# zraorg/ZRA

Measured on AMD Instinct MI355X. Metric: compress + RA-decompress GiB/s, 16 GiB @ 64 KiB frames, 1/2/4/8 MI355X, higher is better.
Workload: dtype u8

## Files before the change

zra_amd/csrc/zra_decode.hip:

```cpp
#include "zra_dev.h"
#include "zra_kernels.h"

using namespace zra_dev;

namespace {

constexpr int DEC_THREADS = 64;
constexpr int BATCH = 64;
#ifndef ZRA_XWIN
#define ZRA_XWIN 4032
#endif
constexpr u32 XPRE = 64, XWIN = ZRA_XWIN;
constexpr u32 BLOCK_MAX = 128u << 10;

__constant__ u32 c_ll_base[36] = {0,1,2,3,4,5,6,7,8,9,10,11,12,13,14,15,16,18,20,22,24,28,32,40,48,64,128,256,512,1024,2048,4096,8192,16384,32768,65536};
__constant__ u8 c_ll_bits[36] = {0,0,0,0,0,0,0,0,0,0,0,0,0,0,0,0,1,1,1,1,2,2,3,3,4,6,7,8,9,10,11,12,13,14,15,16};
__constant__ u32 c_ml_base[53] = {3,4,5,6,7,8,9,10,11,12,13,14,15,16,17,18,19,20,21,22,23,24,25,26,27,28,29,30,31,32,33,34,
                                  35,37,39,41,43,47,51,59,67,83,99,131,259,515,1027,2051,4099,8195,16387,32771,65539};
__constant__ u8 c_ml_bits[53] = {0,0,0,0,0,0,0,0,0,0,0,0,0,0,0,0,0,0,0,0,0,0,0,0,0,0,0,0,0,0,0,0,
                                 1,1,1,1,2,2,3,3,4,4,5,7,8,9,10,11,12,13,14,15,16};
__constant__ short c_ll_defnorm[36] = {4,3,2,2,2,2,2,2,2,2,2,2,2,1,1,1,2,2,2,2,2,2,2,2,2,3,2,1,1,1,1,1,-1,-1,-1,-1};
__constant__ short c_ml_defnorm[53] = {1,4,3,2,2,2,2,2,2,1,1,1,1,1,1,1,1,1,1,1,1,1,1,1,1,1,1,1,1,1,1,1,
                                       1,1,1,1,1,1,1,1,1,1,1,1,1,1,-1,-1,-1,-1,-1,-1,-1};
__constant__ short c_of_defnorm[29] = {1,1,1,1,1,1,2,2,2,1,1,1,1,1,1,1,1,1,1,1,1,1,1,1,-1,-1,-1,-1,-1};
__constant__ u16 c_huf_t0[16][2] = {{0,0},{0,0},{38,130},{448,128},{556,128},{714,128},{883,128},{897,128},{926,128},{947,128},{1107,128},{1177,128},{1242,128},{1349,128},{1455,128},{722,128}};
__constant__ u16 c_huf_t1[16][2] = {{1,1},{1,1},{1313,74},{1353,74},{1353,74},{1418,74},{1437,74},{1515,75},{1613,75},{1729,77},{2083,81},{2379,87},{2415,93},{2644,106},{2422,124},{1891,145}};

__device__ __forceinline__ u64 mk_seqsym(u32 baseValue, u32 addBits, u32 nbBits, u32 nextBase) {
  return (u64)baseValue | ((u64)addBits << 32) | ((u64)nbBits << 40) | ((u64)nextBase << 48);
}
__device__ __forceinline__ u32 mk_cell(u32 sym, u32 addBits, u32 nbBits, u32 nextBase) {
  return sym | (addBits << 8) | (nbBits << 16) | (nextBase << 20);
}

#ifdef ZRA_SMALL_PROFILE
__device__ unsigned long long zra_small_prof[64];
extern "C" __attribute__((visibility("default"))) void ZraHipDebugReadSmallProfile(unsigned long long* out16, int reset) {
  (void)hipMemcpyFromSymbol(out16, HIP_SYMBOL(zra_small_prof), sizeof(unsigned long long) * 64);
  if (reset) { unsigned long long z[64] = {0}; (void)hipMemcpyToSymbol(HIP_SYMBOL(zra_small_prof), z, sizeof(z)); }
}
#define SPROF(k) { __builtin_amdgcn_s_waitcnt(0); const u64 n_ = __builtin_amdgcn_s_memtime(); if (lane == 0) atomicAdd(&zra_small_prof[k], n_ - spt_); spt_ = n_; }
#define SPROF_T0 u64 spt_ = __builtin_amdgcn_s_memtime();
#define SPROF_RESET spt_ = __builtin_amdgcn_s_memtime();
#else
#define SPROF(k)
#define SPROF_T0
#define SPROF_RESET
#endif
#ifdef ZRA_SMALL_PROFILE
#define PPROF_T0 u64 ppt_ = __builtin_amdgcn_s_memtime();
#define PPROF(k) if (FUSED) { __builtin_amdgcn_s_waitcnt(0); const u64 n_ = __builtin_amdgcn_s_memtime(); if (lane == 0) atomicAdd(&zra_small_prof[k], n_ - ppt_); ppt_ = n_; }
#define LPROF_T0 u64 lpt_ = __builtin_amdgcn_s_memtime();
#define LPROF(k) { __builtin_amdgcn_s_waitcnt(0); const u64 n_ = __builtin_amdgcn_s_memtime(); atomicAdd(&zra_small_prof[k], n_ - lpt_); lpt_ = n_; }
#else
#define PPROF_T0
#define PPROF(k)
#define LPROF_T0
#define LPROF(k)
#endif
constexpr u32 STAGE_BYTES = 512;
struct __attribute__((aligned(16))) ParseShared {
  u8 w0[STAGE_BYTES + 16];
  u8 w1[STAGE_BYTES + 16];
  union {
    u64 wt[64];
    u32 stage[1024];
  };
  u16 wnext[256];
  short norm[256];
  u8 spread[512];
  u8 weights[256];
  u16 hufStart[256];
  u32 rankStart[16];
  u32 err, job;
  u32 blkType, blkSize, blkLast, blkPos, hdrPos, frameEnd, winPos, winLen;
  u32 litType, litRegen, litComp, litHdr, litStreams, litRle;
  u32 hufValid, hufMaxBits, hufNSym, hufX2;
  u32 hufNw, hufUsed, hufPhase;
  u32 hufTl, hufMaxSym, hufNcBytes, hufHbyte;
  u32 nbSeq, seqPos, seqModes, seqTables;
  u32 llLog, mlLog, ofLog, llValid, mlValid, ofValid, ofShare;
  u32 rep[3];
  u32 streamOff[4], streamLen[4];
// ... 1185 lines not shown
    const u32 v = (u32)((c << (bc & 63)) >> ((64 - nb) & 63));
    bc += nb; return v;
  }
  __device__ __forceinline__ int reload() {
    if (bc > 64) return OVERFLOW;
    if (ptr >= 8) { ptr -= bc >> 3; bc &= 7; c = fetch(ptr); return UNFINISHED; }
    if (ptr == 0) return bc < 64 ? ENDOFBUFFER : COMPLETED;
    u32 nbBytes = bc >> 3; int r = UNFINISHED;
    if (ptr < nbBytes) { nbBytes = ptr; r = ENDOFBUFFER; }
    ptr -= nbBytes; bc -= nbBytes * 8; c = fetch(ptr);
    return r;
  }
  __device__ __forceinline__ void reload_quiet(bool wide, const u8* pad) {
    const u32 nb = bc <= 64 ? min(bc >> 3, ptr) : 0u;
    ptr -= nb; bc -= nb * 8;
    const u64 v = RING ? fetch(ptr) : ld64(wide ? base + ptr : pad);
    c = nb ? v : c;
  }
};
typedef ZdsT<false> Zds;

}

namespace {
template <bool LDSTAB>
__device__ __forceinline__ void chain_body(const ZraDecodeArgs& a, u32* const ldsTabs, u32* const baseLL, u32* const baseML, u32* const ldsRings = nullptr) {
  const int lane = threadIdx.x;
  const u32 nPend = a.counters[ZRA_DC_NPENDING];
  bool have = false, drained = false;
  ZraDecFrame* F = nullptr;
  const u32* T = nullptr;
  u64* sq = nullptr;
  ZdsT<LDSTAB> br; br.c = 0; br.bc = 0; br.ptr = 0; br.base = nullptr; br.ring = nullptr; br.rLo = 0;
  br.lim = a.body + a.bodySize; br.pf = make_uint4(0, 0, 0, 0); br.pfState = 0; br.pfAge = 0;
  if (LDSTAB) br.ring = (u8*)(ldsRings + (u32)lane * CHAIN_RING_WORDS);
  u32 sLL = 0, sOF = 0, sML = 0, rep0 = 1, rep1 = 4, rep2 = 8;
  u32 i = 0, nbSeq = 0, outPos = 0, litPos = 0, outCap = 0, regen = 0, produced0 = 0, limit = 0;
  u32 longMode = 0, err = 0, jErr = 0xFFFFFFFFu, valid = 0, validOut = 0, validLit = 0, truncated = 0;
  u64 q0 = 0, q1 = 0, q2 = 0;
  u32 eL = 0, eM = 0, eO = 0;
  bool wide = false; const u8* pad = nullptr;
  bool fresh = false; u32 freshJob = 0;
  const u16* const cells16 = (const u16*)ldsTabs + (size_t)lane * ZRA_DEC_TBL_WORDS;
  u32 logLL = 0, logML = 0, logOF = 0;
  auto fetch_cells = [&]() {
    if (LDSTAB) { eL = cells16[ZRA_DEC_TBL_LL + sLL]; eM = cells16[ZRA_DEC_TBL_ML + sML]; eO = cells16[ZRA_DEC_TBL_OF + sOF]; }
    else { eL = T[ZRA_DEC_TBL_LL + sLL]; eM = T[ZRA_DEC_TBL_ML + sML]; eO = T[ZRA_DEC_TBL_OF + sOF]; }
  };
  auto c_code = [&](u32 e) -> u32 { return e & 63u; };
  auto c_sbits = [&](u32 e, u32 lg) -> u32 { if (LDSTAB) return lg - (31u - (u32)__builtin_clz(e >> 6)); return (e >> 16) & 0xF; };
  auto c_sbase = [&](u32 e, u32 lg) -> u32 {
    if (LDSTAB) { const u32 v = e >> 6, hb = 31u - (u32)__builtin_clz(v); return (v ^ (1u << hb)) << (lg - hb); }
    return e >> 20;
  };
  baseLL[lane] = lane < 36 ? c_ll_base[lane] | (LDSTAB ? (u32)c_ll_bits[lane] << 24 : 0u) : 0u;
  baseML[lane] = lane < 53 ? c_ml_base[lane] | (LDSTAB ? (u32)c_ml_bits[lane] << 24 : 0u) : 0u;
  wsync();
  if (LDSTAB && (u32)lane >= ZRA_CHAIN_LDS_FRAMES) drained = true;

  auto finish = [&]() {
    { const u32 r = valid & 3u, b = valid - r;
      if (r >= 1) sq[b] = q0;
      if (r >= 2) sq[b + 1] = q1;
      if (r >= 3) sq[b + 2] = q2; }
    if (!err && !truncated) {
      if (regen - litPos > outCap - outPos) err = ZE_DSTSIZE_TOOSMALL;
    }
    F->chainErr = err; F->nSeqValid = valid; F->seqOut = validOut; F->seqLit = validLit; F->truncated = truncated;
    F->repOut[0] = rep0; F->repOut[1] = rep1; F->repOut[2] = rep2;
    have = false;
  };

  for (;;) {
    const u64 want = __ballot(!have && !drained);
    if (want) {
      u32 base = 0;
      const u32 cnt = (u32)__builtin_popcountll(want);
      if (lane == (int)__builtin_ctzll(want)) base = atomicAdd(&a.counters[ZRA_DC_QCHAIN], cnt);
      base = bcast_u32(base, (u32)__builtin_ctzll(want));
      if (!have && !drained) {
        const u32 idx = base + (u32)__builtin_popcountll(want & ((1ull << lane) - 1ull));
        if (idx >= nPend) drained = true;
        else {
          const u32 j = a.pending[idx];
          const size_t gj = frame_of(a, j);
          F = &a.frames[j];
          T = a.tables + (size_t)j * ZRA_DEC_TBL_WORDS;
          const u8* const blk = a.body + a.frameOff[gj * a.offStride] + F->bpos;
          nbSeq = F->nbSeq; regen = F->litRegen; produced0 = F->produced; longMode = F->longMode;
          outCap = a.outCap[gj] - produced0;
          limit = a.limit ? a.limit[gj] : 0xFFFFFFFFu;
          sq = a.seqs + F->seqBase;
          rep0 = F->rep[0]; rep1 = F->rep[1]; rep2 = F->rep[2];
          i = 0; outPos = 0; litPos = 0; err = 0; jErr = 0xFFFFFFFFu; valid = 0; validOut = 0; validLit = 0; truncated = 0;
          have = true; br.rLo = 0; br.pfState = 0;
          if (F->hufErr) { err = ZE_CORRUPTION; nbSeq = 0; finish(); }
          else if (F->lateErr) { err = F->lateErr; nbSeq = 0; finish(); }
          else if (nbSeq) {
            if (!br.init(blk + F->seqPos, F->bsize - F->seqPos)) { err = ZE_CORRUPTION; finish(); }
            else {
              logLL = F->llLog; logOF = F->ofLog; logML = F->mlLog;
              sLL = br.read(logLL); br.reload();
              sOF = br.read(logOF); br.reload();
              sML = br.read(logML); br.reload();
              wide = F->bsize - F->seqPos >= 8;
              pad = a.body + a.frameOff[gj * a.offStride];
              if (LDSTAB) { fresh = true; freshJob = j; } else fetch_cells();
            }
          }
        }
      }
    }
    if (LDSTAB) {
      u64 nm = __ballot(fresh);
      while (nm) {
        const u32 l = (u32)__builtin_ctzll(nm); nm &= nm - 1;
        const u32 jj = bcast_u32(freshJob, l);
        const uint4* const g4 = (const uint4*)(a.tables + (size_t)jj * ZRA_DEC_TBL_WORDS);
        uint2* const d2 = (uint2*)((u16*)ldsTabs + (size_t)l * ZRA_DEC_TBL_WORDS);
        const ZraDecFrame* const Fj = &a.frames[jj];
        const u32 lgL = Fj->llLog, lgM = Fj->mlLog, lgO = Fj->ofLog;
        for (u32 i = (u32)lane; i < ZRA_DEC_TBL_WORDS / 4; i += DEC_THREADS) {
          const uint4 q = g4[i];
          const u32 lg = 4 * i < ZRA_DEC_TBL_ML ? lgL : 4 * i < ZRA_DEC_TBL_OF ? lgM : lgO;
          auto pk = [&](u32 x) -> u32 { const u32 nb = min((x >> 16) & 0xFu, lg); return (x & 63u) | (((1u << (lg - nb)) | ((x >> 20) >> nb)) << 6); };
          d2[i] = make_uint2(pk(q.x) | (pk(q.y) << 16), pk(q.z) | (pk(q.w) << 16));
        }
      }
      if (__ballot(fresh)) wsync();
      if (fresh) { fetch_cells(); fresh = false; }
    }
    if (!__ballot(have)) break;

    if (have) {
      bool go = true;
      if (LDSTAB) { br.ring_guard(); br.ring_advance(); }
      if (i >= nbSeq) {
        if (!err && nbSeq && !longMode && br.reload() < Zds::COMPLETED) err = ZE_CORRUPTION;
        finish(); go = false;
      } else if (longMode) {
        if (br.reload() > Zds::COMPLETED) {
          if (jErr == 0xFFFFFFFFu || i <= jErr + 4) err = ZE_CORRUPTION;
          finish(); go = false;
        } else if (jErr != 0xFFFFFFFFu && i > jErr + 4) { finish(); go = false; }
      }
      if (go) {
        u32 ll = baseLL[c_code(eL)], ml = baseML[c_code(eM)], off;
        const u32 ofBits = LDSTAB ? c_code(eO) : (eO >> 8) & 0xFF, mlBits = LDSTAB ? ml >> 24 : (eM >> 8) & 0xFF, llBits = LDSTAB ? ll >> 24 : (eL >> 8) & 0xFF;
        if (LDSTAB) { ll &= 0xFFFFFFu; ml &= 0xFFFFFFu; }
        bool badOff = false;
        if (ofBits > 1) {
          off = ((1u << ofBits) - 3u) + br.read_fast(ofBits);
          if (a.bpf > 1 && off >= ZRA_REP_MARK_LO) badOff = true;
          rep2 = rep1; rep1 = rep0; rep0 = off;
        } else {
          const u32 ll0 = (ll == 0);
          if (ofBits == 0) {
            if (!ll0) off = rep0;
            else { off = rep1; rep1 = rep0; rep0 = off; }
          } else {
            const u32 idx = 1 + ll0 + br.read_fast(1);
            u32 t = idx == 3 ? rep0 - 1 : idx == 1 ? rep1 : rep2;
            t += !t;
            if (idx != 1) rep2 = rep1;
            rep1 = rep0; rep0 = off = t;
          }
        }
        if (mlBits) ml += br.read_fast(mlBits);
        if (llBits + mlBits + ofBits >= 57 - (9 + 9 + 8)) br.reload();
        if (llBits) ll += br.read_fast(llBits);
        sLL = c_sbase(eL, logLL) + br.read(c_sbits(eL, logLL));
        sML = c_sbase(eM, logML) + br.read(c_sbits(eM, logML));
        sOF = c_sbase(eO, logOF) + br.read(c_sbits(eO, logOF));
        fetch_cells();
        if (!longMode) br.reload_quiet(wide, pad);
        if (jErr == 0xFFFFFFFFu) {
          u32 e = 0;
          if (ll + ml > outCap - outPos) e = ZE_DSTSIZE_TOOSMALL;
          else if (ll > regen - litPos) e = ZE_CORRUPTION;
          else if (badOff || (off > produced0 + outPos + ll && !(a.bpf > 1 && off >= ZRA_REP_MARK_LO))) e = ZE_CORRUPTION;
          if (e) { jErr = i; err = e; if (!longMode) finish(); }
          else {
            const u64 qv = (u64)ll | ((u64)ml << 18) | ((u64)min(off, 0x0FFFFFFFu) << 36);
            const u32 slot = i & 3u;
            if (slot == 0) q0 = qv; else if (slot == 1) q1 = qv; else if (slot == 2) q2 = qv;
            else { uint4* d4 = (uint4*)(sq + (i - 3)); d4[0] = make_uint4((u32)q0, (u32)(q0 >> 32), (u32)q1, (u32)(q1 >> 32)); d4[1] = make_uint4((u32)q2, (u32)(q2 >> 32), (u32)qv, (u32)(qv >> 32)); }
            outPos += ll + ml; litPos += ll;
            valid = i + 1; validOut = outPos; validLit = litPos;
            if (produced0 + outPos >= limit) { truncated = 1; finish(); }
          }
        }
        i++;
      }
    }
  }
}
}

extern "C" __global__ void __launch_bounds__(DEC_THREADS)
zra_dec_chain_kernel(ZraDecodeArgs a) {
  __shared__ u32 baseLL[64], baseML[64];
  chain_body<false>(a, nullptr, baseLL, baseML);
}
extern "C" __global__ void __launch_bounds__(DEC_THREADS)
zra_dec_chain_lds_kernel(ZraDecodeArgs a) {
  extern __shared__ u32 chainLds[];
  chain_body<true>(a, chainLds + 128, chainLds, chainLds + 64, chainLds + 128 + ZRA_CHAIN_LDS_FRAMES * (ZRA_DEC_TBL_WORDS / 2));
}

namespace {
struct __attribute__((aligned(16))) ExecShared {
  union {
    u8 slot[BATCH][64];
    u8 win[XPRE + XWIN];
  };
  u32 endAt[BATCH];
  u32 matchAt[BATCH];
  u32 job;
};
}

#ifdef ZRA_DEC_PROFILE
__device__ unsigned long long zra_dec_prof[16];
#define XCNT(k, v) { if (lane == 0) atomicAdd(&zra_dec_prof[k], (unsigned long long)(v)); }
#define XTIME(k) { __builtin_amdgcn_s_waitcnt(0); const u64 n_ = __builtin_amdgcn_s_memtime(); if (lane == 0) atomicAdd(&zra_dec_prof[k], n_ - xpt_); xpt_ = n_; }
extern "C" __attribute__((visibility("default"))) void ZraHipDebugReadDecProfile(unsigned long long* out16, int reset) {
  (void)hipMemcpyFromSymbol(out16, HIP_SYMBOL(zra_dec_prof), sizeof(unsigned long long) * 16);
  if (reset) { unsigned long long z[16] = {0}; (void)hipMemcpyToSymbol(HIP_SYMBOL(zra_dec_prof), z, sizeof(z)); }
}
#else
#define XCNT(k, v)
#define XTIME(k)
#endif

namespace {
struct ExecCtx {
  u8* out; const u8* lit; u32 litKind; u8 rleByte;
  u32 outBase, litBase;
  const u8* src; u32 srcSize, produced0, regen;
  bool preValid;
};
__device__ __forceinline__ ExecCtx exec_begin(const ZraDecodeArgs& a, const u32 j, const ZraDecFrame* const F) {
  ExecCtx c;
  const size_t gj = j;
  const u64 so = a.frameOff[gj * a.offStride], se = a.frameOff[gj * a.offStride + 1];
  c.src = a.body + so; c.srcSize = (u32)(se - so);
  c.produced0 = F->produced;
  c.out = a.out + a.outOff[j] + c.produced0;
  c.litKind = F->litKind; c.regen = F->litRegen;
  c.lit = c.litKind == 2 ? a.lits + F->litBase : c.src + F->litArg;
  c.rleByte = (u8)F->litArg;
  c.outBase = 0; c.litBase = 0; c.preValid = false;
  return c;
}
__device__ __forceinline__ void exec_step_global(const ExecCtx& c, ExecShared& S, const u32 ll, const u32 ml, const u32 off, const u32 oStart, const u32 lStart,
                                                 const bool act, const int lane) {
  u8* const out = c.out; const u8* const lit = c.lit; const u32 litKind = c.litKind; const u8 rleByte = c.rleByte;
  const u32 mdst = oStart + ll;
#ifdef ZRA_DEC_PROFILE
  u64 xpt_ = __builtin_amdgcn_s_memtime();
#endif
  {
    u8* op = out + oStart;
    const bool longLit = ll > 32;
    if (!longLit && ll) {
      if (litKind == 1) for (u32 b = 0; b < ll; b++) op[b] = rleByte;
      else copy_le64(op, lit + lStart, ll);
    }
    u64 lm = __ballot(longLit);
    while (lm) {
      const u32 k = (u32)__builtin_ctzll(lm); lm &= lm - 1;
      const u32 jl = bcast_u32(ll, k), jo = bcast_u32(oStart, k), js = bcast_u32(lStart, k);
      if (litKind == 1) fill_bytes(out + jo, rleByte, jl, lane, DEC_THREADS);
      else copy_bytes(out + jo, lit + js, jl, lane, DEC_THREADS);
    }
  }
  wsync();
  XTIME(2)
  {
// ... 593 lines not shown
```

zra_amd/csrc/zra_engine.hip:

```cpp
#include "zra_host.h"
#include "zra_dev.h"
#include "zra_format.h"
#include <algorithm>
#include <atomic>

extern "C" __global__ void zra_dec_parse_kernel(ZraDecodeArgs a);
extern "C" __global__ void zra_dec_huf_kernel(ZraDecodeArgs a);
extern "C" __global__ void zra_dec_chain_kernel(ZraDecodeArgs a);
extern "C" __global__ void zra_dec_chain_lds_kernel(ZraDecodeArgs a);
extern "C" __global__ void zra_dec_exec_kernel(ZraDecodeArgs a);
extern "C" __global__ void zra_dec_parse_all_kernel(ZraDecodeArgs a);
extern "C" __global__ void zra_dec_exec_all_kernel(ZraDecodeArgs a);
extern "C" __global__ void zra_ra_small_kernel(ZraDecodeArgs a, uint32_t* bail, const uint32_t* expect, uint32_t jobBase, unsigned long long* result);

using namespace zra_dev;

namespace zra_fmt {
uint32_t crc32(uint32_t crc, const void* data, size_t n) {
  static uint32_t T[8][256];
  static bool init = false;
  if (!init) {
    for (uint32_t i = 0; i < 256; i++) {
      uint32_t c = i;
      for (int k = 0; k < 8; k++) c = (c & 1) ? (0xEDB88320u ^ (c >> 1)) : (c >> 1);
      T[0][i] = c;
    }
    for (uint32_t i = 0; i < 256; i++)
      for (int t = 1; t < 8; t++) T[t][i] = (T[t - 1][i] >> 8) ^ T[0][T[t - 1][i] & 0xFF];
    init = true;
  }
  const uint8_t* p = (const uint8_t*)data;
  crc = ~crc;
  while (n >= 8) {
    uint32_t a = rd32(p) ^ crc, b = rd32(p + 4);
    crc = T[7][a & 0xFF] ^ T[6][(a >> 8) & 0xFF] ^ T[5][(a >> 16) & 0xFF] ^ T[4][a >> 24] ^
          T[3][b & 0xFF] ^ T[2][(b >> 8) & 0xFF] ^ T[1][(b >> 16) & 0xFF] ^ T[0][b >> 24];
    p += 8; n -= 8;
  }
  while (n--) crc = T[0][(crc ^ *p++) & 0xFF] ^ (crc >> 8);
  return ~crc;
}
}

namespace {

__global__ void zra_jobs_from_seektable_kernel(const u8* table, u32 nFrames, u32 frameSize, u64 total,
                                               u64* frameOff, u64* outOff, u32* expect) {
  u32 i = blockIdx.x * blockDim.x + threadIdx.x;
  if (i <= nFrames) frameOff[i] = seek_entry(table, i);
  if (i < nFrames) {
    u64 o = (u64)i * frameSize;
    outOff[i] = o < total ? o : total;
    expect[i] = (u32)frame_expect(i, frameSize, total);
  }
}

constexpr u32 ZE_SIZE_MISMATCH = 255;
__global__ void zra_xxh64_verify_kernel(const u8* out, const u64* outOff, const u32* expect, const u32* produced, const u32* frameMeta,
                                        u32* status, u32 nFrames) {
  const u32 gid = blockIdx.x * blockDim.x + threadIdx.x;
  const u32 f = gid >> 2; const int j = gid & 3;
  const bool live = f < nFrames && status[f] == 0 && frameMeta[2 * (size_t)f] != 2;
  const bool active = live && frameMeta[2 * (size_t)f] == 1;
  const u8* p = active ? out + outOff[f] : out;
  const u32 n = active ? produced[f] : 0;
  const u64 h = zra_xxh64_quad(p, n, j);
  if (live && j == 0) {
    if (active && (u32)h != frameMeta[2 * (size_t)f + 1]) status[f] = ZE_CHECKSUM_WRONG;
    else if (expect && produced[f] != expect[f]) status[f] = ZE_SIZE_MISMATCH;
  }
}

__global__ void zra_first_error_kernel(const u32* status, u32 nFrames, u32 jobBase, unsigned long long* result) {
  u32 i = blockIdx.x * blockDim.x + threadIdx.x;
  if (i < nFrames && status[i]) atomicMin(result, ((unsigned long long)(jobBase + i) << 8) | (status[i] & 0xFF));
}

}

namespace zra_eng {

static std::atomic<uint64_t> g_scratchBytes{0};
uint64_t scratch_bytes_in_use() { return g_scratchBytes.load(); }

bool DevBuf::reserve(size_t n) {
  if (n <= cap) return true;
  if (p) { (void)hipFree(p); g_scratchBytes -= cap; p = nullptr; cap = 0; }
  size_t want = n + n / 8 + 256;
  static const uint64_t limit = zra_env::env_set("ZRA_ALLOC_LIMIT_MIB") ? (uint64_t)zra_env::env_i64("ZRA_ALLOC_LIMIT_MIB", 0) << 20 : ~0ull;
  const hipError_t ea = want > limit ? hipErrorOutOfMemory : hipMalloc(&p, want);
  if (ea != hipSuccess) { p = nullptr; cap = 0; (void)hipGetLastError(); return false; }
  cap = want; g_scratchBytes += cap;
// ... 6 lines not shown
  if (rd32(b + 8) != kZraMagic || rd16(b + 12) > kVersion) return kHeaderInvalid;
  h->version = rd16(b + 12);
  h->size = rd32(b + 4) + 8;
  h->uncompressedSize = rd64(b + 18);
  h->frameSize = rd32(b + 30);
  h->metaOffset = (uint32_t)kFixedSize;
  h->metaSize = rd32(b + 34);
  h->seekTableOffset = h->metaOffset + h->metaSize;
  h->seekTableSize = rd32(b + 26) * (uint32_t)kEntrySize;
  if (h->version != 1) return kVersionLow;
  return 0;
}

Status Engine::create(Engine** out, int device) {
  int n = 0;
  if (hipGetDeviceCount(&n) != hipSuccess || n <= 0 || device < 0 || device >= n) return zerr(1);
  HIPCHK(hipSetDevice(device));
  Engine* e = new Engine();
  e->device_ = device;
  hipDeviceProp_t prop;
  if (hipGetDeviceProperties(&prop, device) != hipSuccess) { delete e; return zerr(1); }
  e->numCUs_ = prop.multiProcessorCount;
  if (hipStreamCreateWithFlags(&e->stream_, hipStreamNonBlocking) != hipSuccess) { delete e; return zerr(1); }
  {
    int lo = 0, hi = 0;
    if (hipDeviceGetStreamPriorityRange(&lo, &hi) == hipSuccess && hi != lo) {
      if (hipStreamCreateWithPriority(&e->stream2_, hipStreamNonBlocking, hi) != hipSuccess) { delete e; return zerr(1); }
    } else if (hipStreamCreateWithFlags(&e->stream2_, hipStreamNonBlocking) != hipSuccess) { delete e; return zerr(1); }
  }
  if (hipEventCreate(&e->ev0_) != hipSuccess || hipEventCreate(&e->ev1_) != hipSuccess ||
      hipEventCreateWithFlags(&e->evWait_, hipEventDisableTiming) != hipSuccess) { delete e; return zerr(1); }
  for (auto& ev : e->evR_) if (hipEventCreate(&ev) != hipSuccess) { delete e; return zerr(1); }
  *out = e;
  return ok();
}

void Engine::free_scratch() {
  for (DevBuf* b : {&raPlan_, &raLimit_, &raPieceBase_, &raPieces_, &decFrames_, &decTables_, &decLists_, &decCounters_, &decLits_, &decSeqs_, &roundN_, &status_,
                    &produced_, &frameMeta_, &frameOff_, &outOff_, &expect_, &result_, &stage_, &qmeta_, &encScan_, &hostIn_, &hostOut_, &seqScratch_, &mfFlags_, &decBlkRecs_, &decBlkTables_, &decBlkLists_})
    b->release();
  for (auto& x : encCtx_) for (DevBuf* b : {&x.tables, &x.seqs, &x.lits, &x.work, &x.slots, &x.misc, &x.ck, &x.sizes, &x.rec}) b->release();
  for (DevBuf* b : {&upd_.plan, &upd_.packed, &upd_.encSizes, &upd_.frames, &upd_.table, &upd_.copies}) b->release();
  for (DevBuf* b : {&vfy_.plan, &vfy_.faults, &scan_.tables, &scan_.list, &fp_.flags, &fp_.dirty, &fp_.tables, &fp_.list, &rec_.tables, &rec_.ranges}) b->release();
}

Status Engine::release_scratch() {
  HIPCHK(hipSetDevice(device_));
  HIPCHK(hipStreamSynchronize(stream_));
  HIPCHK(hipStreamSynchronize(stream2_));
  free_scratch();
  mfTeleDev_ = nullptr;
  decCountersClean_ = false;
  return ok();
}

Engine::~Engine() {
  (void)hipSetDevice(device_);
  if (stream_) (void)hipStreamSynchronize(stream_);
  free_scratch();
  for (auto ev : evPool_) (void)hipEventDestroy(ev);
  for (auto ev : stageEv_) (void)hipEventDestroy(ev);
  if (stream2_) { (void)hipStreamSynchronize(stream2_); (void)hipStreamDestroy(stream2_); }
  for (auto st : pipeStreams_) if (st) { (void)hipStreamSynchronize(st); (void)hipStreamDestroy(st); }
  if (pinQ_) (void)hipHostFree(pinQ_);
  if (pinSmall_) (void)hipHostFree(pinSmall_);
  for (auto& ev : evR_) if (ev) (void)hipEventDestroy(ev);
  for (auto ev : evCall_) if (ev) (void)hipEventDestroy(ev);
  if (ev0_) (void)hipEventDestroy(ev0_);
  if (ev1_) (void)hipEventDestroy(ev1_);
  if (evWait_) (void)hipEventDestroy(evWait_);
  if (stream_) (void)hipStreamDestroy(stream_);
}

Status Engine::sync() { HIPCHK(hipSetDevice(device_)); HIPCHK(hipStreamSynchronize(stream_)); HIPCHK(hipStreamSynchronize(stream2_)); return ok(); }

Status Engine::wait_stream(hipStream_t producer) {
  HIPCHK(hipSetDevice(device_));
  HIPCHK(hipEventRecord(evWait_, producer));
  HIPCHK(hipStreamWaitEvent(stream_, evWait_, 0));
  HIPCHK(hipStreamWaitEvent(stream2_, evWait_, 0));
  return ok();
}

Status Engine::decode_scratch(ZraDecodeArgs& a, uint32_t maxFrameBytes) {
  const uint32_t n = a.nFrames;
  const uint64_t perFrame = std::min<uint64_t>((uint64_t)maxFrameBytes + 16, (128u << 10) + 16);
  const uint64_t litCap = std::max<uint64_t>((uint64_t)n * perFrame / 2, 1u << 20);
  const uint64_t seqCap = std::max<uint64_t>((uint64_t)n * perFrame * 3 / 32, 1u << 20);
  if (!decFrames_.reserve((size_t)n * sizeof(ZraDecFrame)) || !decTables_.reserve((size_t)n * ZRA_DEC_TBL_WORDS * 4) ||
      !decLists_.reserve((size_t)n * 16 + 64) || !decCounters_.reserve(ZRA_DC_WORDS * 4 + 64) || !decLits_.reserve(litCap + 64) ||
      !decSeqs_.reserve(seqCap * 8 + 64) || !status_.reserve((size_t)n * 4) || !produced_.reserve((size_t)n * 4) ||
      !frameMeta_.reserve((size_t)n * 8) || !result_.reserve(64))
    return zerr(64 );
  uint32_t* listA = decLists_.as<uint32_t>();
  a.pending = listA + 2 * (size_t)n; a.hufJobs = listA + 3 * (size_t)n;
  a.counters = decCounters_.as<uint32_t>();
  a.frames = decFrames_.as<ZraDecFrame>(); a.tables = decTables_.as<uint32_t>();
  a.lits = decLits_.as<uint8_t>(); a.litCap = litCap; a.seqs = decSeqs_.as<uint64_t>(); a.seqCap = seqCap;
  a.status = status_.as<uint32_t>(); a.produced = produced_.as<uint32_t>(); a.frameMeta = frameMeta_.as<uint32_t>();
  return ok();
}

Status Engine::decode_small(const ZraDecodeArgs& a0, const uint32_t* dExpect, uint32_t maxFrameBytes, uint32_t jobBase, unsigned long long* hResult, uint32_t* bailed) {
  ZraDecodeArgs a = a0;
  const uint32_t n = a.nFrames;
  RaTrace trace{"    small", 12};
  { Status st = decode_scratch(a, maxFrameBytes); if (st.zra) return st; }
  trace.mark("scratch");
  a.active = nullptr; a.nActive = n; a.round = 0; a.nextActive = decLists_.as<uint32_t>();
  if (!decCountersClean_) HIPCHK(hipMemsetAsync(a.counters, 0, ZRA_DC_WORDS * 4, stream_));
  decCountersClean_ = false;
  uint32_t* dBail = (uint32_t*)(result_.as<uint8_t>() + 8);
  HIPCHK(hipEventRecord(ev0_, stream_));
  hipLaunchKernelGGL(zra_ra_small_kernel, dim3(n), dim3(192), 0, stream_, a, dBail, dExpect, jobBase, result_.as<unsigned long long>());
  HIPCHK(hipEventRecord(ev1_, stream_));
  trace.mark("launched");
  unsigned long long two[2] = {~0ull, ~0ull};
  HIPCHK(hipMemcpyAsync(two, result_.p, 16, hipMemcpyDeviceToHost, stream_));
  trace.mark("queued rest");
  HIPCHK(hipStreamSynchronize(stream_));
  trace.mark("sync");
  HIPCHK(hipGetLastError());
  if (hipMemsetAsync(a.counters, 0, ZRA_DC_WORDS * 4, stream_) == hipSuccess) decCountersClean_ = true;
  two[1] = 0xFFFFFFFFull - (two[1] & 0xFFFFFFFFull);
  *bailed = (uint32_t)two[1];
  if (!*bailed) *hResult = two[0];
  float ms = 0;
  if (hipEventElapsedTime(&ms, ev0_, ev1_) == hipSuccess) { lastKernelMs_ = ms; kstats_[4] += ms; kstats_[5] += 1; dstats_[5] += ms; dstats_[6] += 1; }
  return ok();
}

hipEvent_t Engine::stage_event() {
  if (stageEvNext_ == stageEv_.size()) { hipEvent_t e = nullptr; if (hipEventCreate(&e) != hipSuccess) return nullptr; stageEv_.push_back(e); }
  return stageEv_[stageEvNext_++];
}

Status Engine::launch_chain(uint64_t nJobs, const ZraDecodeArgs& mid, hipEvent_t after) {
  constexpr uint32_t chainWaves = 2;
  static const uint32_t chainLdsMin = (uint32_t)zra_env::env_int("ZRA_DEC_CHAIN_LDS_MIN", numCUs_ * 96);
  static const int chainLdsMode = zra_env::env_int("ZRA_DEC_CHAIN_LDS", 1);
  const uint32_t gridChain = (uint32_t)std::min<uint64_t>((nJobs + 63) / 64, (uint64_t)numCUs_ * chainWaves);
  if (chainLdsMode != 0 && nJobs >= chainLdsMin) {
    if (!pipeStreams_[1]) { if (hipStreamCreateWithFlags(&pipeStreams_[1], hipStreamNonBlocking) != hipSuccess) { pipeStreams_[1] = nullptr; (void)hipGetLastError(); } }
    const size_t ldsBytes = (128 + (size_t)ZRA_CHAIN_LDS_FRAMES * (ZRA_DEC_TBL_WORDS / 2 + ZRA_CHAIN_RING_WORDS)) * 4;
    if (pipeStreams_[1] && !chainLdsAttr_) {
      if (hipFuncSetAttribute((const void*)zra_dec_chain_lds_kernel, hipFuncAttributeMaxDynamicSharedMemorySize, (int)ldsBytes) == hipSuccess) chainLdsAttr_ = 1;
      else { chainLdsAttr_ = -1; (void)hipGetLastError(); }
    }
    if (pipeStreams_[1] && chainLdsAttr_ > 0) {
      hipEvent_t eJoin = stage_event(); if (!eJoin) return zerr(1);
      HIPCHK(hipStreamWaitEvent(pipeStreams_[1], after, 0));
      hipLaunchKernelGGL(zra_dec_chain_lds_kernel, dim3((uint32_t)numCUs_), dim3(64), ldsBytes, pipeStreams_[1], mid);
      HIPCHK(hipEventRecord(eJoin, pipeStreams_[1]));
      if (chainLdsMode != 2) hipLaunchKernelGGL(zra_dec_chain_kernel, dim3(gridChain), dim3(64), 0, stream_, mid);
      HIPCHK(hipStreamWaitEvent(stream_, eJoin, 0));
      return ok();
    }
  }
  hipLaunchKernelGGL(zra_dec_chain_kernel, dim3(gridChain), dim3(64), 0, stream_, mid);
  return ok();
}

Status Engine::launch_stages(uint64_t nJobs, const ZraDecodeArgs& a, const ZraDecodeArgs& mid, uint32_t nFrames, bool blockPass, hipEvent_t se[5]) {
  for (int k = 0; k < 5; k++) { se[k] = stage_event(); if (!se[k]) return zerr(1); }
  const uint32_t gridParse = (uint32_t)std::min<uint64_t>(nFrames, (uint64_t)numCUs_ * decOccParse_);
  const uint32_t gridHuf = (uint32_t)std::min<uint64_t>((nJobs + ZRA_HUF_FRAMES - 1) / ZRA_HUF_FRAMES, (uint64_t)numCUs_ * decOccHuf_);
  const uint32_t gridExec = (uint32_t)std::min<uint64_t>(nFrames, (uint64_t)numCUs_ * decOccExec_);
  HIPCHK(hipEventRecord(se[0], stream_));
  hipLaunchKernelGGL(blockPass ? zra_dec_parse_all_kernel : zra_dec_parse_kernel, dim3(gridParse), dim3(64), 0, stream_, a);
  HIPCHK(hipEventRecord(se[1], stream_));
  hipLaunchKernelGGL(zra_dec_huf_kernel, dim3(gridHuf), dim3(64), 0, stream_, mid);
  HIPCHK(hipEventRecord(se[2], stream_));
  { Status st = launch_chain(nJobs, mid, se[2]); if (st.zra) return st; }
  HIPCHK(hipEventRecord(se[3], stream_));
  hipLaunchKernelGGL(blockPass ? zra_dec_exec_all_kernel : zra_dec_exec_kernel, dim3(gridExec), dim3(64), 0, stream_, a);
  HIPCHK(hipEventRecord(se[4], stream_));
  return ok();
}

Status Engine::decode_launch(const ZraDecodeArgs& a0, const uint32_t* dExpect, uint32_t maxFrameBytes, uint32_t jobBase, unsigned long long* hResult) {
  ZraDecodeArgs a = a0;
  const uint32_t n = a.nFrames;
  { Status st = decode_scratch(a, maxFrameBytes); if (st.zra) return st; }
  decCountersClean_ = false;
  static const int decFront = zra_env::env_int("ZRA_DEC_FRONT", 1);
  a.decFront = decFront != 0;
  uint32_t* listA = decLists_.as<uint32_t>(); uint32_t* listB = listA + n;
  if (!decOccParse_) {
    HIPCHK(hipOccupancyMaxActiveBlocksPerMultiprocessor(&decOccParse_, zra_dec_parse_kernel, 64, 0));
    HIPCHK(hipOccupancyMaxActiveBlocksPerMultiprocessor(&decOccExec_, zra_dec_exec_kernel, 64, 0));
    HIPCHK(hipOccupancyMaxActiveBlocksPerMultiprocessor(&decOccHuf_, zra_dec_huf_kernel, 64, 0));
    decOccParse_ = std::max(1, decOccParse_); decOccExec_ = std::max(1, decOccExec_); decOccHuf_ = std::max(1, decOccHuf_);
  }
  HIPCHK(hipEventRecord(ev0_, stream_));
  constexpr uint32_t aheadCap = 16;
  if (!roundN_.reserve(4 * (aheadCap + 2) + 64)) return zerr(64);
  static const int fmbEnv = zra_env::env_int("ZRA_DEC_FMB", 1);
  static const uint32_t fmbMin = (uint32_t)zra_env::env_int("ZRA_DEC_FMB_MIN", 64);
  const uint32_t bpf = (uint32_t)(((uint64_t)maxFrameBytes + ZRA_FMB_BLOCK - 1) / ZRA_FMB_BLOCK);
  bool fmb = fmbEnv != 0 && bpf >= 2 && maxFrameBytes <= (64u << 20) && n >= fmbMin && (uint64_t)n * bpf < (1ull << 30);
  uint32_t nRest = n;
  if (fmb) {
    const uint64_t nb = (uint64_t)n * bpf;
    const uint64_t litAll = std::max<uint64_t>((uint64_t)n * ((uint64_t)maxFrameBytes + 16) / 2, 1u << 20);
    const uint64_t seqAll = std::max<uint64_t>((uint64_t)n * ((uint64_t)maxFrameBytes + 16) * 3 / 32, 1u << 20);
    if (!decBlkRecs_.reserve((size_t)nb * sizeof(ZraDecFrame)) || !decBlkTables_.reserve((size_t)nb * ZRA_DEC_TBL_WORDS * 4) ||
        !decBlkLists_.reserve((size_t)(2 * nb + n) * 4 + 64) || !decLits_.reserve(litAll + 64) || !decSeqs_.reserve(seqAll * 8 + 64)) {
      (void)hipGetLastError();
      fmb = false;
    }
    a.lits = decLits_.as<uint8_t>(); a.seqs = decSeqs_.as<uint64_t>();
    if (fmb) {
      ZraDecodeArgs x = a;
      x.bpf = bpf; x.blkRecs = decBlkRecs_.as<ZraDecFrame>(); x.blkTables = decBlkTables_.as<uint32_t>();
      uint32_t* bl = decBlkLists_.as<uint32_t>();
      x.pending = bl; x.hufJobs = bl + nb; x.execList = bl + 2 * nb;
      x.litCap = litAll; x.seqCap = seqAll;
      x.active = nullptr; x.nActive = n; x.round = 0; x.nActivePtr = nullptr; x.nextActive = listA;
      HIPCHK(hipMemsetAsync(x.counters, 0, ZRA_DC_WORDS * 4, stream_));
      ZraDecodeArgs y = x; y.frames = x.blkRecs; y.tables = x.blkTables;
      hipEvent_t se[5];
      { Status st = launch_stages(nb, x, y, n, true, se); if (st.zra) return st; }
      uint32_t back = 0;
      HIPCHK(hipMemcpyAsync(&back, x.counters + ZRA_DC_NNEXT, 4, hipMemcpyDeviceToHost, stream_));
      HIPCHK(hipStreamSynchronize(stream_));
      HIPCHK(hipGetLastError());
      for (int k = 0; k < 4; k++) { float m = 0; if (hipEventElapsedTime(&m, se[k], se[k + 1]) == hipSuccess) dstats_[k] += m; }
      dstats_[4] += 1;
      stageEvNext_ = 0;
      nRest = back;
    }
  }
  auto run_rounds = [&](ZraDecodeArgs& x, uint32_t nActive, const uint32_t* active, uint32_t round, uint32_t* lA, uint32_t* lB, uint32_t ahead) -> Status {
    uint32_t* const dN = roundN_.as<uint32_t>();
    while (nActive) {
      const uint32_t burst = std::max(1u, std::min(ahead, aheadCap));
      hipEvent_t se[aheadCap][5];
      for (uint32_t bi = 0; bi < burst; bi++) {
        HIPCHK(hipMemsetAsync(x.counters, 0, ZRA_DC_WORDS * 4, stream_));
        x.active = active; x.nActive = nActive; x.round = round + bi;
        x.nActivePtr = bi ? dN + bi : nullptr;
        x.nextActive = (active == lA) ? lB : lA;
        { Status st = launch_stages(nActive, x, x, nActive, false, se[bi]); if (st.zra) return st; }
        HIPCHK(hipMemcpyAsync(dN + bi + 1, x.counters + ZRA_DC_NNEXT, 4, hipMemcpyDeviceToDevice, stream_));
        active = x.nextActive;
      }
      uint32_t next = 0;
      HIPCHK(hipMemcpyAsync(&next, dN + burst, 4, hipMemcpyDeviceToHost, stream_));
      HIPCHK(hipStreamSynchronize(stream_));
      HIPCHK(hipGetLastError());
      for (uint32_t bi = 0; bi < burst; bi++)
        for (int k = 0; k < 4; k++) { float m = 0; if (hipEventElapsedTime(&m, se[bi][k], se[bi][k + 1]) == hipSuccess) dstats_[k] += m; }
      dstats_[4] += burst;
      stageEvNext_ = 0;
      x.nActivePtr = nullptr;
      nActive = next; round += burst; ahead = 1;
      if (round > (1u << 20)) return zerr(1);
    }
    return ok();
  };
  Status st = fmb ? run_rounds(a, nRest, listA, 0, listA, listB, 1)
                  : run_rounds(a, n, nullptr, 0, listA, listB, (maxFrameBytes + (128u << 10) - 1) / (128u << 10));
  if (st.zra) return st;
  HIPCHK(hipEventRecord(ev1_, stream_));
  const uint32_t tb = 256;
  hipLaunchKernelGGL(zra_xxh64_verify_kernel, dim3((n * 4 + tb - 1) / tb), dim3(tb), 0, stream_, a.out, a.outOff, dExpect,
                     produced_.as<uint32_t>(), frameMeta_.as<uint32_t>(), status_.as<uint32_t>(), n);
  hipLaunchKernelGGL(zra_first_error_kernel, dim3((n + tb - 1) / tb), dim3(tb), 0, stream_, status_.as<uint32_t>(), n, jobBase,
                     result_.as<unsigned long long>());
  HIPCHK(hipMemcpyAsync(hResult, result_.p, 8, hipMemcpyDeviceToHost, stream_));
  HIPCHK(hipStreamSynchronize(stream_));
  HIPCHK(hipGetLastError());
  float ms = 0;
  if (hipEventElapsedTime(&ms, ev0_, ev1_) == hipSuccess) { lastKernelMs_ = ms; kstats_[4] += ms; kstats_[5] += 1; }
  return ok();
}

Status Engine::decode_pass(const ZraDecodeArgs& b, const uint32_t* dExpect, uint32_t maxFrameBytes, uint32_t jobBase, unsigned long long* res) {
  static const uint32_t smallMax = (uint32_t)zra_env::env_int("ZRA_DEC_SMALL_MAX", 1024);
  if (b.nFrames <= smallMax) {
    uint32_t bailed = 0;
    unsigned long long r2 = *res;
    Status st = decode_small(b, dExpect, maxFrameBytes, jobBase, &r2, &bailed);
    if (st.zra) return st;
    if (!bailed) { *res = r2; return ok(); }
    if (*res == ~0ull) HIPCHK(hipMemsetAsync(result_.p, 0xFF, 64, stream_));
    else { unsigned long long keep = *res; HIPCHK(hipMemsetAsync(result_.p, 0xFF, 64, stream_)); HIPCHK(hipMemcpyAsync(result_.p, &keep, 8, hipMemcpyHostToDevice, stream_)); HIPCHK(hipStreamSynchronize(stream_)); }
  }
  return decode_launch(b, dExpect, maxFrameBytes, jobBase, res);
}

Status Engine::staged_pass(const ArchiveView& a, uint32_t j0, uint32_t n, uint8_t* window, unsigned long long* firstError) {
  lastProducedTotal_ = ~0ull;
  if (!result_.reserve(64)) return zerr(64);
  HIPCHK_CLR(hipMemsetAsync(result_.p, 0xFF, 64, stream_));
  ZraDecodeArgs b{};
  b.body = a.body; b.bodySize = a.bodyBytes; b.out = window; b.offStride = 2; b.nFrames = n;
  b.frameOff = frameOff_.as<uint64_t>() + 2 * (size_t)j0; b.outOff = outOff_.as<uint64_t>(); b.outCap = expect_.as<uint32_t>() + j0;
  *firstError = ~0ull;
// ... 143 lines not shown
```

zra_amd/csrc/zra_kernels.h:

```cpp
#pragma once
#include <stdint.h>
#include <stddef.h>

#ifndef ZRA_HUF_FRAMES
#define ZRA_HUF_FRAMES 2
#endif
#define ZRA_DEC_TBL_LL 0u
#define ZRA_DEC_TBL_ML 512u
#define ZRA_DEC_TBL_OF 1024u
#define ZRA_DEC_TBL_WORDS 1280u
#define ZRA_LDS_TBL_LL 0u
#define ZRA_LDS_TBL_ML 1024u
#define ZRA_LDS_TBL_OF 2048u
#define ZRA_LDS_TBL_WORDS 2304u
#define ZRA_CHAIN_LDS_FRAMES 59u
#define ZRA_CHAIN_RING_WORDS 36u

struct ZraDecFrame {
  uint32_t blkPos, produced, done;
  uint32_t hufValid, hufMaxBits, hufNSym, hufX2;
  uint32_t llValid, mlValid, ofValid, llLog, mlLog, ofLog, ofShare;
  uint32_t rep[3];
  uint32_t fcsLo, fcsHi, fcsHave, hasChecksum, bigWindow;
  uint32_t bpos, bsize, blast;
  uint32_t litKind, litRegen, litArg;
  uint32_t litStreams, streamOff[4], streamLen[4];
  uint32_t hufErr, lateErr;
  uint32_t nbSeq, seqPos, longMode;
  uint64_t litBase, seqBase;
  uint32_t chainErr, nSeqValid, seqOut, seqLit, truncated;
  uint32_t repOut[3];
  uint32_t nBlk, endPos, parseTrunc, pad1_;
  alignas(8) uint8_t weights[256];
  alignas(8) uint16_t hufStart[256];
};
#define ZRA_REP_MARK_LO 0x0C000000u
#define ZRA_REP_MARK(k) (ZRA_REP_MARK_LO + ((uint32_t)(k) << 24) + 0x00800000u)
#define ZRA_FMB_BLOCK (128u << 10)

struct ZraRaPiece { uint64_t dstOff; uint32_t srcOff, len; };

struct RaPlan {
  uint32_t* cnt;
  uint32_t* need;
  uint32_t* slot;
  uint32_t* cursor;
  uint32_t* totals;
  static constexpr size_t kTotalsWords = 16;
  static size_t words(uint32_t nFrames) { return 4 * (size_t)nFrames + kTotalsWords; }
  static RaPlan over(uint32_t* p, uint32_t n) { return RaPlan{p, p + n, p + 2 * (size_t)n, p + 3 * (size_t)n, p + 4 * (size_t)n}; }
  uint32_t* lookup_words() const { return totals + 8; }
};

struct ZraDecodeArgs {
  const uint8_t* body;
  uint64_t bodySize;
  const uint64_t* frameOff;
  uint32_t offStride;
  uint8_t* out;
  const uint64_t* outOff;
  const uint32_t* outCap;
  uint32_t nFrames;
  const uint32_t* limit;
  const uint32_t* pieceBase;
  const ZraRaPiece* pieces;
  uint8_t* raOut;
  const uint32_t* active;
  uint32_t nActive;
  const uint32_t* nActivePtr;
  uint32_t round;
  uint32_t* counters;
  uint32_t* nextActive;
  uint32_t* pending;
  uint32_t* hufJobs;
  ZraDecFrame* frames;
  uint32_t* tables;
  uint8_t* lits; uint64_t litCap;
  uint64_t* seqs; uint64_t seqCap;
  uint32_t* status;
  uint32_t* produced;
  uint32_t* frameMeta;
  uint32_t decFront;
  uint32_t bpf;
  ZraDecFrame* blkRecs;
  uint32_t* blkTables;
  uint32_t* execList;
};
#define ZRA_DC_QPARSE 0
#define ZRA_DC_QCHAIN 1
#define ZRA_DC_QEXEC 2
#define ZRA_DC_NPENDING 3
#define ZRA_DC_NNEXT 4
#define ZRA_DC_NHUF 5
#define ZRA_DC_QHUF 10
#define ZRA_DC_LITCUR 6
#define ZRA_DC_SEQCUR 8
#define ZRA_DC_NEXEC 11
#define ZRA_DC_QEXECALL 12
#define ZRA_DC_WORDS 16

struct ZraEncParams {
  uint32_t windowLog, chainLog, hashLog, searchLog, minMatch, targetLength, strategy;
  uint32_t blockSize;
};

#define ZRA_OPT_NUM 4096u
struct ZraOptCell { int32_t price; uint32_t off, mlen, litlen, rep[3]; };
struct ZraOptMatch { uint32_t off, len; };
struct ZraOptState {
  uint32_t litFreq[256], litLengthFreq[36], matchLengthFreq[53], offCodeFreq[32];
  uint32_t litSum, litLengthSum, matchLengthSum, offCodeSum;
  uint32_t litSumBasePrice, litLengthSumBasePrice, matchLengthSumBasePrice, offCodeSumBasePrice;
  uint32_t predef, pad;
  ZraOptCell table[ZRA_OPT_NUM + 1];
  ZraOptMatch matches[ZRA_OPT_NUM + 1];
};

struct ZraFseCTable {
  uint16_t stateTable[512];
  uint32_t deltaNbBits[53];
  int32_t deltaFindState[53];
  uint32_t tableLog, maxSym, rle;
};

struct alignas(16) ZraEncFrameState {
  uint32_t rep[3];
  uint32_t nextToUpdate;
  uint32_t insEnd;
  uint32_t pad0_[3];
  uint32_t ring[128][4];
  uint32_t idxShift;
  uint32_t outPos;
  uint32_t hufRepeat;
  uint32_t llRepeat, ofRepeat, mlRepeat;
  uint32_t hufMaxSym;
  uint8_t hufNbBits[256];
  uint16_t hufVal[256];
  ZraFseCTable ll, of, ml;
};
static_assert(sizeof(ZraEncFrameState) % 16 == 0 && offsetof(ZraEncFrameState, ring) % 16 == 0, "ZraEncFrameState::ring must be 16-byte aligned in arrays");

struct ZraEntRec {
  ZraFseCTable ct[3];
  uint32_t nChain;
  uint32_t run[3];
  uint32_t finalState[3];
  uint32_t tlog[3];
  uint32_t tblErr;
  uint32_t opOff, lastNCountOff;
  uint32_t newHuf, newHufMaxSym;
  uint32_t pad_;
};

struct ZraEncBlockOut {
  uint32_t nbSeq, lastLL, skip;
  uint32_t rep[3];
  uint32_t ready;
  uint32_t pad_;
};

struct ZraEncArgs {
  const uint8_t* in;
  uint64_t inSize;
  uint32_t frameSize;
  uint32_t firstFrame;
  uint32_t nFrames;
  uint32_t checksum;
  uint32_t mfFilter;
  uint32_t serialAll;
// ... 51 lines not shown
```

Measured before the change: 21.10.

## Sort chain-decode jobs by sequence count before launching chain kernel

Adds a two-phase counting-sort kernel that buckets pending chain jobs by nbSeq (longest first, errored frames last) into a new chainOrder list, which the chain kernel's dynamic work queue now consumes. The aim is longest-job-first scheduling, so big frames start early and tail imbalance across waves shrinks. It costs two extra kernel launches, an event record and scratch for the histogram and order list. An env flag can turn it off.

```diff
diff --git a/zra_amd/csrc/zra_decode.hip b/zra_amd/csrc/zra_decode.hip
--- a/zra_amd/csrc/zra_decode.hip
+++ b/zra_amd/csrc/zra_decode.hip
@@ -1,4 +1,5 @@
 #include "zra_dev.h"
+#include "zra_joblist.h"
 #include "zra_kernels.h"
 
 using namespace zra_dev;
@@ -1350,7 +1351,7 @@
         const u32 idx = base + (u32)__builtin_popcountll(want & ((1ull << lane) - 1ull));
         if (idx >= nPend) drained = true;
         else {
-          const u32 j = a.pending[idx];
+          const u32 j = a.chainOrder[idx];
           const size_t gj = frame_of(a, j);
           F = &a.frames[j];
           T = a.tables + (size_t)j * ZRA_DEC_TBL_WORDS;
@@ -1463,6 +1464,63 @@
     }
   }
 }
+}
+
+extern "C" __global__ void __launch_bounds__(1024)
+zra_dec_chain_order_kernel(ZraDecodeArgs a, u32 phase) {
+  constexpr u32 NC = ZRA_CHAIN_CLASSES, CH = ZRA_CHAIN_ORDER_CHUNK;
+  __shared__ u32 sCnt[NC], sPart[2][32][NC], sAll[NC], sBase[NC];
+  const u32 t = threadIdx.x;
+  const u32 nPend = a.counters[ZRA_DC_NPENDING];
+  const u32 nChunks = (nPend + CH - 1) / CH, per = (nChunks + gridDim.x - 1) / gridDim.x;
+  const u32 c0 = blockIdx.x * per, c1 = min(nChunks, c0 + per);
+  if (c0 >= c1) return;
+  auto class_of = [&](u32 j) -> u32 {
+    const ZraDecFrame* const F = &a.frames[j];
+    return (F->hufErr | F->lateErr) ? 0u : min(F->nbSeq >> 8, NC - 1);
+  };
+  if (phase == 0) {
+    for (u32 ch = c0; ch < c1; ch++) {
+      if (t < NC) sCnt[t] = 0;
+      __syncthreads();
+      const u32 i = ch * CH + t;
+      if (i < nPend) atomicAdd(&sCnt[class_of(a.pending[i])], 1u);
+      __syncthreads();
+      if (t < NC) a.chainHist[(size_t)ch * NC + t] = sCnt[t];
+    }
+    return;
+  }
+  {
+    const u32 c = t & (NC - 1), g = t / NC;
+    u32 before = 0, all = 0;
+    for (u32 ch = g; ch < nChunks; ch += 32) { const u32 v = a.chainHist[(size_t)ch * NC + c]; all += v; if (ch < c0) before += v; }
+    sPart[0][g][c] = before; sPart[1][g][c] = all;
+  }
+  __syncthreads();
+  if (t < NC) {
+    u32 before = 0, all = 0;
+    for (u32 g = 0; g < 32; g++) { before += sPart[0][g][t]; all += sPart[1][g][t]; }
+    sBase[t] = before; sAll[t] = all;
+  }
+  __syncthreads();
+  if (t < NC) { u32 higher = 0; for (u32 k = t + 1; k < NC; k++) higher += sAll[k]; sBase[t] += higher; }
+  __syncthreads();
+  for (u32 ch = c0; ch < c1; ch++) {
+    const u32 i = ch * CH + t;
+    const bool in = i < nPend;
+    const u32 j = in ? a.pending[i] : 0u, cls = in ? class_of(j) : NC;
+    bool p[NC]; u32 rank[NC], total[NC];
+#pragma unroll
+    for (u32 c = 0; c < NC; c++) p[c] = cls == c;
+    block_rank<(int)NC>(p, rank, total);
+    u32 r = 0, tot = 0;
+#pragma unroll
+    for (u32 c = 0; c < NC; c++) { if (cls == c) r = rank[c]; if (t == c) tot = total[c]; }
+    if (in) a.chainOrder[sBase[cls] + r] = j;
+    __syncthreads();
+    if (t < NC) sBase[t] += tot;
+    __syncthreads();
+  }
 }
 
 extern "C" __global__ void __launch_bounds__(DEC_THREADS)
diff --git a/zra_amd/csrc/zra_engine.hip b/zra_amd/csrc/zra_engine.hip
--- a/zra_amd/csrc/zra_engine.hip
+++ b/zra_amd/csrc/zra_engine.hip
@@ -8,6 +8,7 @@
 extern "C" __global__ void zra_dec_huf_kernel(ZraDecodeArgs a);
 extern "C" __global__ void zra_dec_chain_kernel(ZraDecodeArgs a);
 extern "C" __global__ void zra_dec_chain_lds_kernel(ZraDecodeArgs a);
+extern "C" __global__ void zra_dec_chain_order_kernel(ZraDecodeArgs a, uint32_t phase);
 extern "C" __global__ void zra_dec_exec_kernel(ZraDecodeArgs a);
 extern "C" __global__ void zra_dec_parse_all_kernel(ZraDecodeArgs a);
 extern "C" __global__ void zra_dec_exec_all_kernel(ZraDecodeArgs a);
@@ -180,18 +181,21 @@
   return ok();
 }
 
+static size_t chain_hist_words(uint64_t nJobs) { return (size_t)(nJobs / ZRA_CHAIN_ORDER_CHUNK + 1) * ZRA_CHAIN_CLASSES; }
+
 Status Engine::decode_scratch(ZraDecodeArgs& a, uint32_t maxFrameBytes) {
   const uint32_t n = a.nFrames;
   const uint64_t perFrame = std::min<uint64_t>((uint64_t)maxFrameBytes + 16, (128u << 10) + 16);
   const uint64_t litCap = std::max<uint64_t>((uint64_t)n * perFrame / 2, 1u << 20);
   const uint64_t seqCap = std::max<uint64_t>((uint64_t)n * perFrame * 3 / 32, 1u << 20);
   if (!decFrames_.reserve((size_t)n * sizeof(ZraDecFrame)) || !decTables_.reserve((size_t)n * ZRA_DEC_TBL_WORDS * 4) ||
-      !decLists_.reserve((size_t)n * 16 + 64) || !decCounters_.reserve(ZRA_DC_WORDS * 4 + 64) || !decLits_.reserve(litCap + 64) ||
+      !decLists_.reserve(((size_t)n * 5 + chain_hist_words(n)) * 4 + 64) || !decCounters_.reserve(ZRA_DC_WORDS * 4 + 64) || !decLits_.reserve(litCap + 64) ||
       !decSeqs_.reserve(seqCap * 8 + 64) || !status_.reserve((size_t)n * 4) || !produced_.reserve((size_t)n * 4) ||
       !frameMeta_.reserve((size_t)n * 8) || !result_.reserve(64))
     return zerr(64 );
   uint32_t* listA = decLists_.as<uint32_t>();
   a.pending = listA + 2 * (size_t)n; a.hufJobs = listA + 3 * (size_t)n;
+  a.chainOrder = listA + 4 * (size_t)n; a.chainHist = listA + 5 * (size_t)n;
   a.counters = decCounters_.as<uint32_t>();
   a.frames = decFrames_.as<ZraDecFrame>(); a.tables = decTables_.as<uint32_t>();
   a.lits = decLits_.as<uint8_t>(); a.litCap = litCap; a.seqs = decSeqs_.as<uint64_t>(); a.seqCap = seqCap;
@@ -233,7 +237,16 @@
   return stageEv_[stageEvNext_++];
 }
 
-Status Engine::launch_chain(uint64_t nJobs, const ZraDecodeArgs& mid, hipEvent_t after) {
+Status Engine::launch_chain(uint64_t nJobs, const ZraDecodeArgs& mid0, hipEvent_t after) {
+  static const bool ordered = zra_env::env_int("ZRA_DEC_CHAIN_PREP", 1) != 0;
+  ZraDecodeArgs mid = mid0;
+  if (ordered) {
+    const uint32_t gridOrder = (uint32_t)std::min<uint64_t>(std::max<uint64_t>(1, (nJobs + ZRA_CHAIN_ORDER_CHUNK - 1) / ZRA_CHAIN_ORDER_CHUNK), (uint64_t)numCUs_);
+    hipLaunchKernelGGL(zra_dec_chain_order_kernel, dim3(gridOrder), dim3(1024), 0, stream_, mid, 0u);
+    hipLaunchKernelGGL(zra_dec_chain_order_kernel, dim3(gridOrder), dim3(1024), 0, stream_, mid, 1u);
+    after = stage_event(); if (!after) return zerr(1);
+    HIPCHK(hipEventRecord(after, stream_));
+  } else mid.chainOrder = mid.pending;
   constexpr uint32_t chainWaves = 2;
   static const uint32_t chainLdsMin = (uint32_t)zra_env::env_int("ZRA_DEC_CHAIN_LDS_MIN", numCUs_ * 96);
   static const int chainLdsMode = zra_env::env_int("ZRA_DEC_CHAIN_LDS", 1);
@@ -303,7 +316,7 @@
     const uint64_t litAll = std::max<uint64_t>((uint64_t)n * ((uint64_t)maxFrameBytes + 16) / 2, 1u << 20);
     const uint64_t seqAll = std::max<uint64_t>((uint64_t)n * ((uint64_t)maxFrameBytes + 16) * 3 / 32, 1u << 20);
     if (!decBlkRecs_.reserve((size_t)nb * sizeof(ZraDecFrame)) || !decBlkTables_.reserve((size_t)nb * ZRA_DEC_TBL_WORDS * 4) ||
-        !decBlkLists_.reserve((size_t)(2 * nb + n) * 4 + 64) || !decLits_.reserve(litAll + 64) || !decSeqs_.reserve(seqAll * 8 + 64)) {
+        !decBlkLists_.reserve(((size_t)(3 * nb + n) + chain_hist_words(nb)) * 4 + 64) || !decLits_.reserve(litAll + 64) || !decSeqs_.reserve(seqAll * 8 + 64)) {
       (void)hipGetLastError();
       fmb = false;
     }
@@ -313,6 +326,7 @@
       x.bpf = bpf; x.blkRecs = decBlkRecs_.as<ZraDecFrame>(); x.blkTables = decBlkTables_.as<uint32_t>();
       uint32_t* bl = decBlkLists_.as<uint32_t>();
       x.pending = bl; x.hufJobs = bl + nb; x.execList = bl + 2 * nb;
+      x.chainOrder = bl + 2 * nb + n; x.chainHist = bl + 3 * nb + n;
       x.litCap = litAll; x.seqCap = seqAll;
       x.active = nullptr; x.nActive = n; x.round = 0; x.nActivePtr = nullptr; x.nextActive = listA;
       HIPCHK(hipMemsetAsync(x.counters, 0, ZRA_DC_WORDS * 4, stream_));
diff --git a/zra_amd/csrc/zra_kernels.h b/zra_amd/csrc/zra_kernels.h
--- a/zra_amd/csrc/zra_kernels.h
+++ b/zra_amd/csrc/zra_kernels.h
@@ -15,6 +15,8 @@
 #define ZRA_LDS_TBL_WORDS 2304u
 #define ZRA_CHAIN_LDS_FRAMES 59u
 #define ZRA_CHAIN_RING_WORDS 36u
+#define ZRA_CHAIN_CLASSES 32u
+#define ZRA_CHAIN_ORDER_CHUNK 1024u
 
 struct ZraDecFrame {
   uint32_t blkPos, produced, done;
@@ -85,6 +87,8 @@
   ZraDecFrame* blkRecs;
   uint32_t* blkTables;
   uint32_t* execList;
+  uint32_t* chainOrder;
+  uint32_t* chainHist;
 };
 #define ZRA_DC_QPARSE 0
 #define ZRA_DC_QCHAIN 1
```

Measured after the change: 20.75. -1.7%, worse.
